# KLab/YAIK

Measured on AMD Instinct MI355X. Metric: Mpix/s tile encode (alpha reject + 7 gradient passes + 8x8 range quant), 8K RGBA, higher is better.
Workload: dtype u8/int32 (+f32 mode-selection sums)

## Files before the change

yaik_amd/csrc/yk_encode2.hip:

```cpp
#include "yk_common.h"
#include "yk_curves.h"
#include "yk_device.h"
#include <mutex>

__constant__ float c_curve2[6][16] = YK_CURVE_TABLE;

#define LS YK_LSTRIDE
#ifdef YK_TEST_HOOKS
#define YK2_ABLATE(bit) ((P.ablate & (bit)) != 0)
#else
#define YK2_ABLATE(bit) false
#endif

__device__ __forceinline__ int y2_byte(uint32_t w, int ch) { return (w >> (8 * ch)) & 255; }
__device__ __forceinline__ uint32_t y2_absdiff(uint32_t a, uint32_t b) { uint32_t r; asm("v_sad_u32 %0, %1, %2, 0" : "=v"(r) : "v"(a), "v"(b)); return r; }
__device__ __forceinline__ int y2_round6(int v) { return (v & ~3) | (v >> 6); }
__device__ __forceinline__ int y2_round6p(int v) { v = min(v + 1, 255); return (v & ~3) | (v >> 6); }

typedef short y2s2 __attribute__((ext_vector_type(2)));
typedef unsigned short y2u2 __attribute__((ext_vector_type(2)));
__device__ __forceinline__ y2u2 y2_u2(uint32_t w) { return __builtin_bit_cast(y2u2, w); }
__device__ __forceinline__ y2s2 y2_s2(y2u2 v) { return __builtin_bit_cast(y2s2, v); }
__device__ __forceinline__ y2u2 y2_splat(int v) { const unsigned short t = (unsigned short)v; return (y2u2){ t, t }; }
__device__ __forceinline__ y2s2 y2_splats(int v) { const short t = (short)v; return (y2s2){ t, t }; }
#define YK2_LATN 85
#ifdef YK2_STATS
__device__ unsigned long long g_y2_stats[128];
#define YK2_STAT(i, n) do { if (lane == 0) atomicAdd(&g_y2_stats[(i)], (unsigned long long)(n)); } while (0)
extern "C" int yk_debug_path_stats(unsigned long long* out, int clear) {
    hipError_t e = hipMemcpyFromSymbol(out, HIP_SYMBOL(g_y2_stats), sizeof(g_y2_stats));
    if (e == hipSuccess && clear) { static unsigned long long z[128]; e = hipMemcpyToSymbol(HIP_SYMBOL(g_y2_stats), z, sizeof(z)); }
    return (int)e;
}
#else
#define YK2_STAT(i, n) do { } while (0)
#endif

__device__ __forceinline__ constexpr int y2_cell_x(int m) { return (m & 1) | ((m >> 1) & 2); }
__device__ __forceinline__ constexpr int y2_cell_y(int m) { return ((m >> 1) & 1) | ((m >> 2) & 2); }
template <int NX, int NY> __device__ __forceinline__ constexpr unsigned long long y2_origin() {
    unsigned long long m = 0;
    for (int i = 0; i < 16; i++) if ((y2_cell_x(i) % NX) == 0 && (y2_cell_y(i) % NY) == 0) m |= 1ULL << i;
    return m * 0x0001000100010001ULL;
}
template <int NX, int NY> __device__ __forceinline__ unsigned long long y2_fold(unsigned long long m) {
    if (NX >= 2) m |= m >> 1;
    if (NY >= 2) m |= m >> 2;
    if (NX == 4) m |= m >> 4;
    if (NY == 4) m |= m >> 8;
    return m;
}
template <int NX, int NY> __device__ __forceinline__ unsigned long long y2_spread(unsigned long long m) {
    if (NX >= 2) m |= m << 1;
    if (NY >= 2) m |= m << 2;
    if (NX == 4) m |= m << 4;
    if (NY == 4) m |= m << 8;
    return m;
}

template <int SX, int SY, bool SMOOTH = false>
__device__ __forceinline__ void y2_grad_pass(const uint32_t* s_lat, const int lat, const int cx, const int cy,
                                             const uint32_t (&pwb)[16], unsigned long long& cov, const unsigned long long deadLanes, const bool stripInside,
                                             const int gxCell, const int gyCell, const int w, const int h, const int rf,
                                             uint32_t* s_bm, const int bxCell, const int byCell, const uint32_t* s_pix, uint8_t* s_list, uint32_t* s_tf, const int lane) {
    constexpr int TX = 1 << SX, TY = 1 << SY, NX = TX / 4, NY = TY / 4;
    constexpr unsigned long long ORG = y2_origin<NX, NY>();
    const int dcx = cx & (NX - 1), dcy = cy & (NY - 1);
    unsigned long long viable = ORG & ~cov & ~y2_fold<NX, NY>(deadLanes);
    if (!stripInside) {
        const int tgx = gxCell - dcx * 4, tgy = gyCell - dcy * 4;
        viable &= __ballot((tgx + TX <= w) && (tgy + TY <= h));
    }
    if (viable == 0ULL) return;
    constexpr int kPassId = (SX == 4 && SY == 4) ? 0 : (SX == 4 && SY == 3) ? 1 : (SX == 3 && SY == 4) ? 2 : (SX == 3 && SY == 3) ? 3 : (SX == 3 && SY == 2) ? 4 : (SX == 2 && SY == 3) ? 5 : 6;
    YK2_STAT(kPassId * 10 + 0, 1); YK2_STAT(kPassId * 10 + 8, __popcll(y2_spread<NX, NY>(viable)));
    const int loO = -256 * rf, hiO = 256 * rf + 255;
    const y2s2 loO2 = y2_splats(loO), hiO2 = y2_splats(hiO), loR2 = y2_splats(loO - 127), hiR2 = y2_splats(hiO - 127);


#ifndef YK2_NO_COMPACT
    const unsigned long long cells = y2_spread<NX, NY>(viable);
    const int nCells = __popcll(cells);
    if (nCells <= 16) {
        YK2_STAT(kPassId * 10 + 1, 1); YK2_STAT(kPassId * 10 + 7, nCells);
        const int rank = (int)__builtin_amdgcn_mbcnt_hi((uint32_t)(cells >> 32), __builtin_amdgcn_mbcnt_lo((uint32_t)cells, 0u));
        const bool mine = __builtin_amdgcn_inverse_ballot_w64(cells);
        if (mine) s_list[rank] = (uint8_t)lane;
        s_tf[lane] = 0u; s_tf[64 + lane] = 0u;
        __builtin_amdgcn_fence(__ATOMIC_RELEASE, "wavefront"); __builtin_amdgcn_wave_barrier(); __builtin_amdgcn_fence(__ATOMIC_ACQUIRE, "wavefront");
        const int j = lane & 15, r = lane >> 4;
        const bool act = j < nCells;
        const int c = (int)s_list[act ? j : 0];
        const int q2 = c >> 4, cy2 = y2_cell_y(c & 15), cx2 = y2_cell_x(c & 15);
        const int dcx2 = cx2 & (NX - 1), dcy2 = cy2 & (NY - 1);
        constexpr int kInTile = (NX > 1 ? 1 : 0) | (NY > 1 ? 2 : 0) | (NX > 2 ? 4 : 0) | (NY > 2 ? 8 : 0);
        const int orig = c & ~kInTile;
        const int lo2 = cy2 * 17 + q2 * 4 + cx2 - dcy2 * 17 - dcx2;
        const y2u2 wyr = y2_splat(16 - ((dcy2 * 4 + r) << (4 - SY)));
        const y2u2 lxc = y2_splat(16 - ((dcx2 * 4) << (4 - SX)));
        const uint4 pr = *reinterpret_cast<const uint4*>(&s_pix[(cy2 * 4 + r) * LS + q2 * 16 + cx2 * 4]);
        const uint32_t px[4] = { pr.x ^ 0x00808080u, pr.y ^ 0x00808080u, pr.z ^ 0x00808080u, pr.w ^ 0x00808080u };
        y2s2 mnc[5], mxc[5];
        auto rowC = [&](const unsigned mask) {
            y2u2 Sc[5], stc[5];
#pragma unroll
            for (int t = 0; t < 5; t++) {
                if (!((mask >> t) & 1u)) continue;
                const uint32_t* lt = s_lat + t * YK2_LATN + lo2;
                const y2u2 TL = y2_u2(lt[0]), TR = y2_u2(lt[NX]), BL = y2_u2(lt[NY * 17]), BR = y2_u2(lt[NY * 17 + NX]);
                const y2u2 e16 = (BL - BR) << 4, g = TR - BR, f = TL - BL - g;
                const y2u2 c2 = (g << 4) + f * lxc;
                Sc[t] = ((BR << 8) + e16 * lxc + c2 * wyr) ^ y2_splat(0x8000);
                stc[t] = (e16 + f * wyr) << (4 - SX);
            }
#pragma unroll
            for (int i = 0; i < 4; i++) {
                const uint32_t p = px[i];
                const y2s2 c01 = y2_s2(y2_u2(__builtin_amdgcn_perm(0u, p, 0x010C000Cu))), c22 = y2_s2(y2_u2(__builtin_amdgcn_perm(0u, p, 0x020C020Cu)));
                const y2s2 cc[4] = { __builtin_shufflevector(c01, c01, 0, 0), __builtin_shufflevector(c01, c01, 1, 1), c22, c01 };
#pragma unroll
                for (int t = 0; t < 5; t++) {
                    if (!((mask >> t) & 1u)) continue;
                    const y2s2 D = __builtin_elementwise_sub_sat(y2_s2(Sc[t]), cc[t == 4 ? 2 : t]);
                    if (i == 0) { mnc[t] = D; mxc[t] = D; }
                    else { mnc[t] = __builtin_elementwise_min(mnc[t], D); mxc[t] = __builtin_elementwise_max(mxc[t], D); }
                    if (i < 3) Sc[t] = Sc[t] - stc[t];
                }
            }
        };
        constexpr uint32_t kAllFail = 0xE000E000u;
        auto failBits = [&](const y2s2 mnA, const y2s2 mxA, const y2s2 mnP, const y2s2 mxP) -> uint32_t {
            const y2s2 zero = y2_splats(0);
            const y2s2 oA = __builtin_elementwise_sub_sat(zero, __builtin_elementwise_max(__builtin_elementwise_sub_sat(loO2, mnA), __builtin_elementwise_sub_sat(mxA, hiO2)));
            const y2s2 rA = __builtin_elementwise_sub_sat(zero, __builtin_elementwise_max(__builtin_elementwise_sub_sat(loR2, mnA), __builtin_elementwise_sub_sat(mxA, hiR2)));
            const y2s2 oP = __builtin_elementwise_sub_sat(zero, __builtin_elementwise_max(__builtin_elementwise_sub_sat(loO2, mnP), __builtin_elementwise_sub_sat(mxP, hiO2)));
            const y2s2 rP = __builtin_elementwise_sub_sat(zero, __builtin_elementwise_max(__builtin_elementwise_sub_sat(loR2, mnP), __builtin_elementwise_sub_sat(mxP, hiR2)));
            const uint32_t a = __builtin_bit_cast(uint32_t, oA), b = __builtin_bit_cast(uint32_t, rA), cO = __builtin_bit_cast(uint32_t, oP), cR = __builtin_bit_cast(uint32_t, rP);
            uint32_t m = (a & 0x80008000u) | ((b >> 1) & 0x40004000u);
            m |= (((cO << 16) | cO) >> 2) & 0x20000000u;
            m |= (((cR >> 16) | cR) >> 2) & 0x00002000u;
            return m;
        };
        rowC(0x09u);
        if (act) atomicOr(&s_tf[orig], failBits(mnc[0], mxc[0], mnc[3], mxc[3]));
        __builtin_amdgcn_fence(__ATOMIC_RELEASE, "wavefront"); __builtin_amdgcn_wave_barrier(); __builtin_amdgcn_fence(__ATOMIC_ACQUIRE, "wavefront");
        const unsigned long long alive = viable & __ballot(s_tf[lane] != kAllFail);
        if (alive == 0ULL) { YK2_STAT(100 + kPassId, 1); return; }
        rowC(0x16u);
        {
            const y2s2 mnA = __builtin_elementwise_min(__builtin_elementwise_min(mnc[0], mnc[1]), mnc[2]), mxA = __builtin_elementwise_max(__builtin_elementwise_max(mxc[0], mxc[1]), mxc[2]);
            const y2s2 mnP = __builtin_elementwise_min(mnc[3], mnc[4]), mxP = __builtin_elementwise_max(mxc[3], mxc[4]);
            if (act) atomicOr(&s_tf[64 + orig], failBits(mnA, mxA, mnP, mxP));
        }
        __builtin_amdgcn_fence(__ATOMIC_RELEASE, "wavefront"); __builtin_amdgcn_wave_barrier(); __builtin_amdgcn_fence(__ATOMIC_ACQUIRE, "wavefront");
        const unsigned long long acceptC = alive & __ballot(s_tf[64 + lane] != kAllFail);
        if (acceptC != 0ULL) {
            YK2_STAT(110 + kPassId, 1);
            cov |= y2_spread<NX, NY>(acceptC);
            if (__builtin_amdgcn_inverse_ballot_w64(acceptC)) {
                const int tbx = bxCell >> SX, tby = byCell >> SY;
                int bit;
                if (SX == 4 && SY == 4) bit = 0 + tby * 4 + tbx;
                else if (SX == 4 && SY == 3) bit = 32 + tby * 4 + tbx;
                else if (SX == 3 && SY == 4) bit = 64 + tby * 8 + tbx;
                else if (SX == 3 && SY == 3) bit = 96 + tby * 8 + tbx;
                else if (SX == 3 && SY == 2) bit = 160 + (tby >> 3) * 64 + (tby & 7) * 8 + tbx;
                else if (SX == 2 && SY == 3) bit = 288 + (tbx >> 3) * 64 + tby * 8 + (tbx & 7);
                else bit = 416 + ((tby >> 3) * 2 + (tbx >> 3)) * 64 + (tby & 7) * 8 + (tbx & 7);
                atomicOr(&s_bm[bit >> 5], 1u << (bit & 31));
            }
        }
        return;
    }
#endif

    const int lo = lat - dcy * 17 - dcx;
    const y2u2 wy2 = y2_splat(16 - ((dcy * 4) << (4 - SY)));
    const y2u2 lx2 = y2_splat(16 - ((dcx * 4) << (4 - SX)));
    y2u2 S[5], st[5], dS0[5], dS3[5], dst[5];
    auto setup = [&](const int t) {
        const uint32_t* lt = s_lat + t * YK2_LATN + lo;
        const y2u2 TL = y2_u2(lt[0]), TR = y2_u2(lt[NX]), BL = y2_u2(lt[NY * 17]), BR = y2_u2(lt[NY * 17 + NX]);
        const y2u2 e16 = (BL - BR) << 4, g = TR - BR, f = TL - BL - g;
        const y2u2 c2 = (g << 4) + f * lx2;
        S[t] = ((BR << 8) + e16 * lx2 + c2 * wy2) ^ y2_splat(0x8000);
        dS0[t] = c2 << (4 - SY);
        st[t] = (e16 + f * wy2) << (4 - SX);
        dst[t] = f << (8 - SX - SY);
        dS3[t] = dS0[t] - dst[t] * (unsigned short)3;
    };
    y2s2 mn[5], mx[5];
    auto pixelRow = [&](const int r, const unsigned mask, const bool first) {
#pragma unroll
        for (int ii = 0; ii < 4; ii++) {
            const int i = (r & 1) ? 3 - ii : ii;
            const uint32_t p = pwb[r * 4 + i];
            const y2s2 c01 = y2_s2(y2_u2(__builtin_amdgcn_perm(0u, p, 0x010C000Cu))), c22 = y2_s2(y2_u2(__builtin_amdgcn_perm(0u, p, 0x020C020Cu)));
            const y2s2 cc[4] = { __builtin_shufflevector(c01, c01, 0, 0), __builtin_shufflevector(c01, c01, 1, 1), c22, c01 };
#pragma unroll
            for (int t = 0; t < 5; t++) {
                if (!((mask >> t) & 1u)) continue;
                const y2s2 D = __builtin_elementwise_sub_sat(y2_s2(S[t]), cc[t == 4 ? 2 : t]);
                if (first && ii == 0) { mn[t] = D; mx[t] = D; }
                else { mn[t] = __builtin_elementwise_min(mn[t], D); mx[t] = __builtin_elementwise_max(mx[t], D); }
                if (ii < 3) S[t] = (r & 1) ? S[t] + st[t] : S[t] - st[t];
            }
        }
    };
    auto nextRow = [&](const int r, const unsigned mask) {
#pragma unroll
        for (int t = 0; t < 5; t++) if ((mask >> t) & 1u) { S[t] -= (r & 1) ? dS0[t] : dS3[t]; st[t] -= dst[t]; }
    };
    auto failA4 = [&](const y2s2 mnA, const y2s2 mxA) -> unsigned long long {
        const y2s2 oA = __builtin_elementwise_max(__builtin_elementwise_sub_sat(loO2, mnA), __builtin_elementwise_sub_sat(mxA, hiO2));
        const y2s2 rA = __builtin_elementwise_max(__builtin_elementwise_sub_sat(loR2, mnA), __builtin_elementwise_sub_sat(mxA, hiR2));
        unsigned long long f = y2_fold<NX, NY>(__ballot(oA.x > 0));
        f &= y2_fold<NX, NY>(__ballot(oA.y > 0));
        f &= y2_fold<NX, NY>(__ballot(rA.x > 0));
        f &= y2_fold<NX, NY>(__ballot(rA.y > 0));
        return f;
    };
    auto failP2 = [&](const y2s2 mnP, const y2s2 mxP) -> unsigned long long {
        const y2s2 oP = __builtin_elementwise_max(__builtin_elementwise_sub_sat(loO2, mnP), __builtin_elementwise_sub_sat(mxP, hiO2));
        const y2s2 rP = __builtin_elementwise_max(__builtin_elementwise_sub_sat(loR2, mnP), __builtin_elementwise_sub_sat(mxP, hiR2));
        return y2_fold<NX, NY>(__ballot((oP.x > 0) | (oP.y > 0))) & y2_fold<NX, NY>(__ballot((rP.x > 0) | (rP.y > 0)));
    };
    auto mnAll = [&]() { return __builtin_elementwise_min(__builtin_elementwise_min(mn[0], mn[1]), mn[2]); };
    auto mxAll = [&]() { return __builtin_elementwise_max(__builtin_elementwise_max(mx[0], mx[1]), mx[2]); };

    constexpr bool kScreen = (NX * NY >= 4);
    constexpr unsigned kA = 0x07u, kP = 0x18u;
    unsigned long long accept;
    if (SMOOTH) {
        setup(0); setup(1); setup(2);
        pixelRow(0, kA, true);
        nextRow(0, kA); pixelRow(1, kA, false);
        nextRow(1, kA); pixelRow(2, kA, false);
        nextRow(2, kA); pixelRow(3, kA, false);
        YK2_STAT(kPassId * 10 + 4, 1);
        accept = viable & ~failA4(mnAll(), mxAll());
#ifdef YK2_STATS
        {
            y2u2 S_[5], st_[5], a_[5], b_[5], c_[5]; y2s2 mn_[5], mx_[5];
            for (int t = 0; t < 5; t++) { S_[t] = S[t]; st_[t] = st[t]; a_[t] = dS0[t]; b_[t] = dS3[t]; c_[t] = dst[t]; mn_[t] = mn[t]; mx_[t] = mx[t]; }
            setup(3); setup(4);
            pixelRow(0, kP, true); nextRow(0, kP); pixelRow(1, kP, false); nextRow(1, kP); pixelRow(2, kP, false); nextRow(2, kP); pixelRow(3, kP, false);
            const unsigned long long accP = viable & ~failP2(__builtin_elementwise_min(mn[3], mn[4]), __builtin_elementwise_max(mx[3], mx[4]));
            YK2_STAT(97, __popcll(accept)); YK2_STAT(98, __popcll(accP)); YK2_STAT(99, __popcll(accept | accP)); YK2_STAT(96 + 0 * kPassId, 0);
            YK2_STAT(107, __popcll(viable));
            for (int t = 0; t < 5; t++) { S[t] = S_[t]; st[t] = st_[t]; dS0[t] = a_[t]; dS3[t] = b_[t]; dst[t] = c_[t]; mn[t] = mn_[t]; mx[t] = mx_[t]; }
        }
#endif
        const unsigned long long rest = viable & ~accept;
        if (rest != 0ULL) {
            YK2_STAT(kPassId * 10 + 5, 1); YK2_STAT(90 + kPassId, __popcll(y2_spread<NX, NY>(rest)));
            setup(3);
            pixelRow(0, 0x08u, true);
            const unsigned long long left = rest & ~failP2(mn[3], mx[3]);
            if (left != 0ULL) {
                setup(4);
                pixelRow(0, 0x10u, true);
                nextRow(0, kP); pixelRow(1, kP, false);
                nextRow(1, kP); pixelRow(2, kP, false);
                nextRow(2, kP); pixelRow(3, kP, false);
                accept |= left & ~failP2(__builtin_elementwise_min(mn[3], mn[4]), __builtin_elementwise_max(mx[3], mx[4]));
            }
        }
    } else {
    int pRows;
    if (kScreen) {
        setup(0); setup(3);
        pixelRow(0, 0x09u, true);
        viable &= ~(failA4(mn[0], mx[0]) & failP2(mn[3], mx[3]));
        if (viable == 0ULL) { YK2_STAT(kPassId * 10 + 2, 1); return; }
        setup(1); setup(2);
        pixelRow(0, 0x06u, true);
        viable &= ~(failA4(mnAll(), mxAll()) & failP2(mn[3], mx[3]));
        if (viable == 0ULL) { YK2_STAT(kPassId * 10 + 3, 1); return; }
        nextRow(0, kA);
        pixelRow(1, kA, false);
        pRows = 0;
    } else {
#pragma unroll
        for (int t = 0; t < 5; t++) setup(t);
        pixelRow(0, 0x1Fu, true);
        viable &= ~(failA4(mnAll(), mxAll()) & failP2(__builtin_elementwise_min(mn[3], mn[4]), __builtin_elementwise_max(mx[3], mx[4])));
        if (viable == 0ULL) { YK2_STAT(kPassId * 10 + 3, 1); return; }
        nextRow(0, 0x1Fu);
        pixelRow(1, 0x1Fu, false);
        if (NX * NY == 1) {
            viable &= ~(failA4(mnAll(), mxAll()) & failP2(__builtin_elementwise_min(mn[3], mn[4]), __builtin_elementwise_max(mx[3], mx[4])));
            if (viable == 0ULL) { YK2_STAT(kPassId * 10 + 9, 1); return; }
        }
        pRows = 2;
    }
    YK2_STAT(kPassId * 10 + 4, 1);
    nextRow(1, kA);
    pixelRow(2, kA, false);
    nextRow(2, kA);
    pixelRow(3, kA, false);
    accept = viable & ~failA4(mnAll(), mxAll());
    const unsigned long long rest = viable & ~accept;
    if (rest != 0ULL) {
        YK2_STAT(kPassId * 10 + 5, 1); YK2_STAT(90 + kPassId, __popcll(y2_spread<NX, NY>(rest)));
        if (kScreen) {
            setup(4);
            pixelRow(0, 0x10u, true);
            nextRow(0, kP);
            pixelRow(1, kP, false);
        }
        nextRow(1, kP);
        pixelRow(2, kP, false);
        nextRow(2, kP);
        pixelRow(3, kP, false);
        accept |= rest & ~failP2(__builtin_elementwise_min(mn[3], mn[4]), __builtin_elementwise_max(mx[3], mx[4]));
    }
    (void)pRows;
    }
    if (accept == 0ULL) return;
    YK2_STAT(kPassId * 10 + 6, 1);
    cov |= y2_spread<NX, NY>(accept);
    if (__builtin_amdgcn_inverse_ballot_w64(accept)) {
        const int tbx = bxCell >> SX, tby = byCell >> SY;
        int bit;
        if (SX == 4 && SY == 4) bit = 0 + tby * 4 + tbx;
        else if (SX == 4 && SY == 3) bit = 32 + tby * 4 + tbx;
        else if (SX == 3 && SY == 4) bit = 64 + tby * 8 + tbx;
        else if (SX == 3 && SY == 3) bit = 96 + tby * 8 + tbx;
        else if (SX == 3 && SY == 2) bit = 160 + (tby >> 3) * 64 + (tby & 7) * 8 + tbx;
        else if (SX == 2 && SY == 3) bit = 288 + (tbx >> 3) * 64 + tby * 8 + (tbx & 7);
        else bit = 416 + ((tby >> 3) * 2 + (tbx >> 3)) * 64 + (tby & 7) * 8 + (tbx & 7);
        atomicOr(&s_bm[bit >> 5], 1u << (bit & 31));
    }
}

#define YK2_QROWS 258
#define YK2_QR0 32
#define YK2_QNR 224
#define YK2_QBYTES ((size_t)YK2_QNR * YK2_QROWS * 16)
#define YK2_RCPBYTES ((size_t)256 * sizeof(float))
#define YK2_DEFN1 224
#define YK2_DEFBYTES ((size_t)225 * YK2_DEFN1 * 4)
#define YK2_TABBYTES (YK2_QBYTES + YK2_RCPBYTES + YK2_DEFBYTES)
typedef _Float16 y2h2 __attribute__((ext_vector_type(2)));
__device__ __forceinline__ uint32_t y2_f16_bits(int n) { const _Float16 h = (_Float16)(float)n; return (uint32_t)__builtin_bit_cast(unsigned short, h); }
__global__ void yk_qtab_kernel(uint4* tab) {
    __shared__ int K[6][16];
    const int R = YK2_QR0 + (int)blockIdx.x, t = threadIdx.x;
    if (t < 96) { const int m = t >> 4, i = t & 15; K[m][i] = __float2int_rz(__fmul_rn(c_curve2[m][i], (float)R)); }
    __syncthreads();
    if (t < YK2_QROWS) {
        const int o = t - 2;
        uint32_t md[6], idx = 0;
        for (int m = 0; m < 6; m++) {
            const int cnt = m < 3 ? 16 : 8;
            int best = 1 << 30, bi = 0;
            for (int n = 0; n < cnt; n++) { const int d = abs(K[m][n] - o); if (d < best) { best = d; bi = n; } }
            best = min(best, 255);
            md[m] = y2_f16_bits(best);
            idx |= (uint32_t)bi << (4 * m);
        }
        tab[(size_t)blockIdx.x * YK2_QROWS + t] = make_uint4(md[0] | (md[1] << 16), md[2] | (md[3] << 16), md[4] | (md[5] << 16), idx);
    }
}
struct Y2TileDef { int base, BN, dist, R; };
__device__ __forceinline__ Y2TileDef y2_tile_def(const int min_, const int d8) {
    Y2TileDef d;
    d.base = (min_ * 63 + 112) / 224;
    d.BN = (d.base * 224) / 63;
    const int scale = 223 - d.BN;
    const int dnum = (d8 - 32) * 127 + (scale - 1);
    d.dist = (scale < 0) ? -dnum : dnum / scale;
    d.R = (d.dist * scale) / 127 + 32;
// ... 193 lines not shown
            Rb = *reinterpret_cast<const int4*>(b0 + off);
            Gb = *reinterpret_cast<const int4*>(b1 + off);
            Bb = *reinterpret_cast<const int4*>(b2 + off);
        }
        uint32_t hcol;
        const int hr = min(max(lane - 32, 0), 16);
        {
            const int rel = min(gyS + hr, P.hAvail - 1) - gyB;
            const uint32_t off = (uint32_t)(rel * P.strideElems + min(BX * 64 + 64, w - 1)) * 4u;
            hcol = y2_pack3(*reinterpret_cast<const int32_t*>(b0 + off), *reinterpret_cast<const int32_t*>(b1 + off), *reinterpret_cast<const int32_t*>(b2 + off));
        }
        const float4 rc4 = *reinterpret_cast<const float4*>(P.qtab + YK2_QBYTES + (size_t)lane * 16);

        __builtin_amdgcn_s_setprio(0);
        uint4 o[4], ob;
#pragma unroll
        for (int k = 0; k < 4; k++) {
            o[k] = make_uint4(y2_pack3(R[k].x, G[k].x, B[k].x), y2_pack3(R[k].y, G[k].y, B[k].y), y2_pack3(R[k].z, G[k].z, B[k].z), y2_pack3(R[k].w, G[k].w, B[k].w));
            *reinterpret_cast<uint4*>(&s_pix[(r0 + 4 * k) * LS + g4]) = o[k];
        }
        ob = make_uint4(y2_pack3(Rb.x, Gb.x, Bb.x), y2_pack3(Rb.y, Gb.y, Bb.y), y2_pack3(Rb.z, Gb.z, Bb.z), y2_pack3(Rb.w, Gb.w, Bb.w));
        if (lane < 16) *reinterpret_cast<uint4*>(&s_pix[16 * LS + g4]) = ob;
        if (BX * 64 + 64 > w) {
            if (!inX) {
#pragma unroll
                for (int k = 0; k < 4; k++) *reinterpret_cast<uint4*>(&s_pix[(r0 + 4 * k) * LS + g4]) = make_uint4(o[k].w, o[k].w, o[k].w, o[k].w);
                if (lane < 16) *reinterpret_cast<uint4*>(&s_pix[16 * LS + g4]) = make_uint4(ob.w, ob.w, ob.w, ob.w);
            }
        }
        if (lane >= 32 && lane <= 48) s_pix[hr * LS + 64] = hcol;
        *reinterpret_cast<float4*>(&s_rcp[lane * 4]) = rc4;

    }
    __syncthreads();
    YK2_PROBE(1);

    const int q = lane >> 4, cx = y2_cell_x(lane & 15), cy = y2_cell_y(lane & 15);
    const int bxCell = q * 16 + cx * 4, byCell = wave * 16 + cy * 4;
    const int gxCell = BX * 64 + bxCell, gyCell = BY * 64 + byCell;
    const int lcell = (cy * 4) * LS + bxCell;
    const int lat = cy * 17 + q * 4 + cx;
    const bool mtIn = (BX * 64 + q * 16 < w) && (BY * 64 + wave * 16 < h);

    uint32_t pw[16];
#pragma unroll
    for (int r = 0; r < 4; r++) {
        const uint4 t = *reinterpret_cast<const uint4*>(&s_pix[lcell + r * LS]);
        pw[r * 4 + 0] = t.x; pw[r * 4 + 1] = t.y; pw[r * 4 + 2] = t.z; pw[r * 4 + 3] = t.w;
    }

    unsigned long long cov = 0ULL;
    {
        bool dead = !mtIn;
        {
            const int lim = 4 * P.rejectFactor + 1;
            const y2u2 rb0 = y2_u2(pw[0] & 0x00FF00FFu), rb1 = y2_u2(pw[1] & 0x00FF00FFu), rb2 = y2_u2(pw[2] & 0x00FF00FFu), rb3 = y2_u2(pw[3] & 0x00FF00FFu);
            const y2u2 ga = y2_u2(__builtin_amdgcn_perm(pw[1], pw[0], 0x0C050C01u)), gb = y2_u2(__builtin_amdgcn_perm(pw[2], pw[1], 0x0C050C01u)),
                       gc = y2_u2(__builtin_amdgcn_perm(pw[3], pw[2], 0x0C050C01u));
            const y2u2 l2 = y2_splat(lim);
            const y2u2 u1 = rb0 + rb2 - rb1 - rb1 + l2, u2 = rb1 + rb3 - rb2 - rb2 + l2, ug = ga + gc - gb - gb + l2;
            const y2u2 um = __builtin_elementwise_max(__builtin_elementwise_max(u1, u2), ug);
            dead |= __builtin_bit_cast(uint32_t, __builtin_elementwise_sub_sat(um, y2_splat(2 * lim))) != 0u;
        }
        const unsigned long long deadLanes = __ballot(dead);
        YK2_STAT(75, 1); YK2_STAT(76, ~deadLanes == 0ULL ? 1 : 0); YK2_STAT(77, __popcll(deadLanes));
        const bool stripInside = (BX * 64 + 64 <= w) && (BY * 64 + wave * 16 + 16 <= h);
        if (~deadLanes != 0ULL && !YK2_ABLATE(2)) {
            auto latticePoint = [&](const int idx) {
                const int lr = (idx * 241) >> 12, lc = idx - lr * 17;
                const uint32_t raw = s_pix[(lr * 4) * LS + lc * 4];
                const uint32_t r6 = (raw & 0x00FCFCFCu) | ((raw >> 6) & 0x00030303u);
                const uint32_t z = (raw & 0x007F7F7Fu) + 0x00010101u;
                const uint32_t inc = (z ^ (raw & 0x00808080u)) | (((z & raw & 0x00808080u) >> 7) * 255u);
                const uint32_t p6 = (inc & 0x00FCFCFCu) | ((inc >> 6) & 0x00030303u);
                s_lat[0 * YK2_LATN + idx] = __builtin_amdgcn_perm(r6, raw, 0x0C040C00u);
                s_lat[1 * YK2_LATN + idx] = __builtin_amdgcn_perm(r6, raw, 0x0C050C01u);
                s_lat[2 * YK2_LATN + idx] = __builtin_amdgcn_perm(r6, raw, 0x0C060C02u);
                s_lat[3 * YK2_LATN + idx] = __builtin_amdgcn_perm(p6, p6, 0x0C010C00u);
                s_lat[4 * YK2_LATN + idx] = __builtin_amdgcn_perm(p6, p6, 0x0C020C02u);
            };
            latticePoint(lane);
            if (lane < YK2_LATN - 64) latticePoint(lane + 64);
            __syncthreads();
#pragma unroll
            for (int k = 0; k < 16; k++) pw[k] ^= 0x00808080u;
            if (deadLanes == 0ULL) y2_grad_pass<4, 4, true>(s_lat, lat, cx, cy, pw, cov, deadLanes, stripInside, gxCell, gyCell, w, h, P.rejectFactor, s_bm, bxCell, byCell, s_pix, s_list, s_range, lane);
            else y2_grad_pass<4, 4>(s_lat, lat, cx, cy, pw, cov, deadLanes, stripInside, gxCell, gyCell, w, h, P.rejectFactor, s_bm, bxCell, byCell, s_pix, s_list, s_range, lane);
            if (~(cov | deadLanes) != 0ULL) {
                y2_grad_pass<4, 3>(s_lat, lat, cx, cy, pw, cov, deadLanes, stripInside, gxCell, gyCell, w, h, P.rejectFactor, s_bm, bxCell, byCell, s_pix, s_list, s_range, lane);
                y2_grad_pass<3, 4>(s_lat, lat, cx, cy, pw, cov, deadLanes, stripInside, gxCell, gyCell, w, h, P.rejectFactor, s_bm, bxCell, byCell, s_pix, s_list, s_range, lane);
                y2_grad_pass<3, 3>(s_lat, lat, cx, cy, pw, cov, deadLanes, stripInside, gxCell, gyCell, w, h, P.rejectFactor, s_bm, bxCell, byCell, s_pix, s_list, s_range, lane);
                y2_grad_pass<3, 2>(s_lat, lat, cx, cy, pw, cov, deadLanes, stripInside, gxCell, gyCell, w, h, P.rejectFactor, s_bm, bxCell, byCell, s_pix, s_list, s_range, lane);
                y2_grad_pass<2, 3>(s_lat, lat, cx, cy, pw, cov, deadLanes, stripInside, gxCell, gyCell, w, h, P.rejectFactor, s_bm, bxCell, byCell, s_pix, s_list, s_range, lane);
                y2_grad_pass<2, 2>(s_lat, lat, cx, cy, pw, cov, deadLanes, stripInside, gxCell, gyCell, w, h, P.rejectFactor, s_bm, bxCell, byCell, s_pix, s_list, s_range, lane);
            }
#pragma unroll
            for (int k = 0; k < 16; k++) pw[k] ^= 0x00808080u;
        }
    }
    const int mtIdx = ((BY * 64 + wave * 16) >> 4) * P.mtW + ((BX * 64 + q * 16) >> 4);
    __syncthreads();
    YK2_PROBE(2);
    uint8_t* const small = P.small;
    const uint32_t bmv = s_bm[lane < 24 ? lane : 0];
    auto bmWord = [&](const int k) -> uint32_t { return (uint32_t)__builtin_amdgcn_readlane((int)bmv, k); };
    const uint32_t i64 = (uint32_t)(BY * P.xBB64 + BX);
    const uint32_t frU = (uint32_t)fr;
    uint32_t off32 = ~0u, val32 = 0u;
    {
        const uint32_t w1 = (uint32_t)wave & 1u, w2 = (uint32_t)wave >> 1;
        uint32_t off8 = 0u, val8 = 0u;
        off8 = y2_writelane(P.oBm0b + frU * (uint32_t)P.fs.bm0b + i64 * 4u + (uint32_t)wave, 0, off8);
        val8 = y2_writelane((bmWord(0) >> (4 * wave)) & 0xFu, 0, val8);
        off8 = y2_writelane(P.oBm[1] + frU * (uint32_t)P.fs.bitmap[1] + i64 * 4u + (uint32_t)wave, 1, off8);
        val8 = y2_writelane(bmWord(1) >> (8 * wave), 1, val8);
        off8 = y2_writelane(P.oBm[2] + frU * (uint32_t)P.fs.bitmap[2] + i64 * 4u + (uint32_t)wave, 2, off8);
        val8 = y2_writelane(bmWord(2) >> (8 * wave), 2, val8);
        if (lane < 3) Y2_STORE_IF(8, *(small + off8), (uint8_t)val8);
        const unsigned long long t = ((cov >> 2) ^ cov) & 0x0C0C0C0C0C0C0C0CULL;
        const unsigned long long covRM = cov ^ t ^ (t << 2);
        uint32_t off16 = ((lane & 15) == 0 && mtIn) ? P.oCov + (frU * (uint32_t)P.fs.coverage + (uint32_t)mtIdx) * 2u : ~0u;
        uint32_t val16 = (uint32_t)((covRM >> (q * 16)) & 0xFFFFULL);
        off16 = y2_writelane(P.oBm[3] + frU * (uint32_t)P.fs.bitmap[3] + (i64 * 4u + (uint32_t)wave) * 2u, 1, off16);
        val16 = y2_writelane(bmWord(3 + (int)w2) >> (16 * w1), 1, val16);
#pragma unroll
        for (int sx = 0; sx < 2; sx++) {
            const bool in = BX * 2 + sx < P.xBB32;
            off16 = y2_writelane(in ? P.oBm[5] + frU * (uint32_t)P.fs.bitmap[5] + ((uint32_t)((BY * P.xBB32 + BX * 2 + sx) * 4 + wave)) * 2u : ~0u, 2 + sx, off16);
            val16 = y2_writelane(bmWord(9 + sx * 2 + (int)w2) >> (16 * w1), 2 + sx, val16);
        }
        if (off16 != ~0u) Y2_STORE_IF(8, *reinterpret_cast<uint16_t*>(small + off16), (uint16_t)val16);
        if (P.pixCache != nullptr) {
            const bool cellIn = (gxCell < w) && (gyCell < h);
            if (cellIn && !((cov >> lane) & 1ULL)) {
                const uint32_t strip = (uint32_t)((BY * 4 + wave) * P.xBB64 + BX);
                uint4* dstp = P.pixCache + (size_t)strip * 256 + lane;
#pragma unroll
                for (int r = 0; r < 4; r++) dstp[r * 64] = make_uint4(pw[r * 4 + 0], pw[r * 4 + 1], pw[r * 4 + 2], pw[r * 4 + 3]);
            }
        }
        {
            const bool in = BY * 2 + (int)w2 < P.yBB32;
            off32 = y2_writelane(in ? P.oBm[4] + frU * (uint32_t)P.fs.bitmap[4] + ((uint32_t)(((BY * 2 + (int)w2) * P.xBB64 + BX) * 2) + w1) * 4u : ~0u, 1, off32);
            val32 = y2_writelane(bmWord(5 + (int)w2 * 2 + (int)w1), 1, val32);
#pragma unroll
            for (int sx = 0; sx < 2; sx++) {
                const bool in6 = in && (BX * 2 + sx < P.xBB32);
                off32 = y2_writelane(in6 ? P.oBm[6] + frU * (uint32_t)P.fs.bitmap[6] + ((uint32_t)(((BY * 2 + (int)w2) * P.xBB32 + BX * 2 + sx) * 2) + w1) * 4u : ~0u, 2 + sx, off32);
                val32 = y2_writelane(bmWord(13 + ((int)w2 * 2 + sx) * 2 + (int)w1), 2 + sx, val32);
            }
        }
    }
    YK2_PROBE(3);
    int cxB = 0, cyB = 0, cw = w, chh = P.fullH, discard = 1;
    if (boundsP) {
        const int b0 = boundsP[0], b1 = boundsP[1], b2 = boundsP[2], b3 = boundsP[3];
        discard = (b0 == 0 && b1 == 0 && b2 == w && b3 == P.fullH) ? 1 : 0;
        cxB = (b0 >> 3) << 3; cyB = (b1 >> 3) << 3;
        cw = (((b2 + 7) >> 3) << 3) - cxB; chh = (((b3 + 7) >> 3) << 3) - cyB;
    }
    const int cxl = cx & 1, cyl = cy & 1;
    const int tgx = gxCell - cxl * 4, tgyl = gyCell - cyl * 4, tgy = tgyl + P.y0;
    const bool tileIn = (tgx + 8 <= w) && (tgyl + 8 <= h);
    const bool part = tileIn && tgx >= cxB && tgx < cxB + cw && tgy >= cyB && tgy < cyB + chh && (tgx + 8 <= cw) && (tgy + 8 <= chh);
    const bool keepMT = (keepP == nullptr) || discard || (mtIn && keepP[mtIdx] != 0);
    const bool tileLive = part && keepMT;
    const int l00 = lane & ~3;
    const uint32_t quadN = (uint32_t)((~cov) >> l00) & 15u;
    const int v00 = (int)(quadN & 1u), v01 = (int)((quadN >> 2) & 1u);
    const bool valid = tileLive && ((quadN >> (lane & 3)) & 1u);
    const int nTop = __popc(quadN & 3u), nBot = __popc(quadN >> 2);
    const int tileIdx = (tgyl >> 3) * P.tilesW + (tgx >> 3);
    const size_t T8 = (size_t)P.tilesW * P.tilesH;
    const int tw = lane >> 2;
    const bool writer = ((lane & 3) == 0) && tileIn;
    const unsigned long long validMask = __ballot(valid);
#ifdef YK2_NO_WIDE_STORE
    const bool fullTiles = false;
#else
    const bool fullTiles = !WANT_DST && __ballot(tileLive && quadN != 15u && quadN != 0u) == 0ULL;
// ... 418 lines not shown
```

Baseline: 227,800.

## Pre-unpack pixel channels once and pack blue-channel pass two pixels per lane

Pixels are unpacked into signed 16-bit RG and paired-blue vectors once per tile and passed to every gradient pass, so each pass no longer repeats the perm/xor unpack. The fifth term (blue, which was duplicated) is now evaluated for two pixels per packed op, using precomputed per-half start and row-step values, which halves its per-pixel instruction count. The early two-row reject check is extended to passes with NX*NY equal to 2. The cost is extra registers for the 24 pre-unpacked vectors plus a reload of pw from LDS afterwards, which may raise VGPR pressure and lower occupancy.

```diff
diff --git a/yaik_amd/csrc/yk_encode2.hip b/yaik_amd/csrc/yk_encode2.hip
--- a/yaik_amd/csrc/yk_encode2.hip
+++ b/yaik_amd/csrc/yk_encode2.hip
@@ -23,6 +23,8 @@
 __device__ __forceinline__ y2s2 y2_s2(y2u2 v) { return __builtin_bit_cast(y2s2, v); }
 __device__ __forceinline__ y2u2 y2_splat(int v) { const unsigned short t = (unsigned short)v; return (y2u2){ t, t }; }
 __device__ __forceinline__ y2s2 y2_splats(int v) { const short t = (short)v; return (y2s2){ t, t }; }
+__device__ __forceinline__ y2s2 y2_rg(uint32_t p) { return y2_s2(y2_u2(__builtin_amdgcn_perm(0u, p, 0x010C000Cu) ^ 0x80008000u)); }
+__device__ __forceinline__ y2s2 y2_bb(uint32_t pEven, uint32_t pOdd) { return y2_s2(y2_u2(__builtin_amdgcn_perm(pOdd, pEven, 0x060C020Cu) ^ 0x80008000u)); }
 #define YK2_LATN 85
 #ifdef YK2_STATS
 __device__ unsigned long long g_y2_stats[128];
@@ -60,7 +62,7 @@
 
 template <int SX, int SY, bool SMOOTH = false>
 __device__ __forceinline__ void y2_grad_pass(const uint32_t* s_lat, const int lat, const int cx, const int cy,
-                                             const uint32_t (&pwb)[16], unsigned long long& cov, const unsigned long long deadLanes, const bool stripInside,
+                                             const y2s2 (&rg)[16], const y2s2 (&bb)[8], unsigned long long& cov, const unsigned long long deadLanes, const bool stripInside,
                                              const int gxCell, const int gyCell, const int w, const int h, const int rf,
                                              uint32_t* s_bm, const int bxCell, const int byCell, const uint32_t* s_pix, uint8_t* s_list, uint32_t* s_tf, const int lane) {
     constexpr int TX = 1 << SX, TY = 1 << SY, NX = TX / 4, NY = TY / 4;
@@ -99,7 +101,7 @@
         const y2u2 wyr = y2_splat(16 - ((dcy2 * 4 + r) << (4 - SY)));
         const y2u2 lxc = y2_splat(16 - ((dcx2 * 4) << (4 - SX)));
         const uint4 pr = *reinterpret_cast<const uint4*>(&s_pix[(cy2 * 4 + r) * LS + q2 * 16 + cx2 * 4]);
-        const uint32_t px[4] = { pr.x ^ 0x00808080u, pr.y ^ 0x00808080u, pr.z ^ 0x00808080u, pr.w ^ 0x00808080u };
+        const y2s2 rgc[4] = { y2_rg(pr.x), y2_rg(pr.y), y2_rg(pr.z), y2_rg(pr.w) }, bbc[2] = { y2_bb(pr.x, pr.y), y2_bb(pr.z, pr.w) };
         y2s2 mnc[5], mxc[5];
         auto rowC = [&](const unsigned mask) {
             y2u2 Sc[5], stc[5];
@@ -115,17 +117,22 @@
             }
 #pragma unroll
             for (int i = 0; i < 4; i++) {
-                const uint32_t p = px[i];
-                const y2s2 c01 = y2_s2(y2_u2(__builtin_amdgcn_perm(0u, p, 0x010C000Cu))), c22 = y2_s2(y2_u2(__builtin_amdgcn_perm(0u, p, 0x020C020Cu)));
-                const y2s2 cc[4] = { __builtin_shufflevector(c01, c01, 0, 0), __builtin_shufflevector(c01, c01, 1, 1), c22, c01 };
-#pragma unroll
-                for (int t = 0; t < 5; t++) {
+                const y2s2 c01 = rgc[i], cb = bbc[i >> 1];
+                const y2s2 cc[4] = { __builtin_shufflevector(c01, c01, 0, 0), __builtin_shufflevector(c01, c01, 1, 1),
+                                     (i & 1) ? __builtin_shufflevector(cb, cb, 1, 1) : __builtin_shufflevector(cb, cb, 0, 0), c01 };
+#pragma unroll
+                for (int t = 0; t < 4; t++) {
                     if (!((mask >> t) & 1u)) continue;
-                    const y2s2 D = __builtin_elementwise_sub_sat(y2_s2(Sc[t]), cc[t == 4 ? 2 : t]);
+                    const y2s2 D = __builtin_elementwise_sub_sat(y2_s2(Sc[t]), cc[t]);
                     if (i == 0) { mnc[t] = D; mxc[t] = D; }
                     else { mnc[t] = __builtin_elementwise_min(mnc[t], D); mxc[t] = __builtin_elementwise_max(mxc[t], D); }
                     if (i < 3) Sc[t] = Sc[t] - stc[t];
                 }
+            }
+            if (mask & 0x10u) {
+                const y2s2 Da = __builtin_elementwise_sub_sat(y2_s2(Sc[4] - stc[4] * (y2u2){ 0, 1 }), bbc[0]);
+                const y2s2 Db = __builtin_elementwise_sub_sat(y2_s2(Sc[4] - stc[4] * (y2u2){ 2, 3 }), bbc[1]);
+                mnc[4] = __builtin_elementwise_min(Da, Db); mxc[4] = __builtin_elementwise_max(Da, Db);
             }
         };
         constexpr uint32_t kAllFail = 0xE000E000u;
@@ -177,39 +184,55 @@
     const int lo = lat - dcy * 17 - dcx;
     const y2u2 wy2 = y2_splat(16 - ((dcy * 4) << (4 - SY)));
     const y2u2 lx2 = y2_splat(16 - ((dcx * 4) << (4 - SX)));
-    y2u2 S[5], st[5], dS0[5], dS3[5], dst[5];
+    y2u2 S[4], st[4], dS0[4], dS3[4], dst[4], Sa, Sb, rsA, rsB;
     auto setup = [&](const int t) {
         const uint32_t* lt = s_lat + t * YK2_LATN + lo;
         const y2u2 TL = y2_u2(lt[0]), TR = y2_u2(lt[NX]), BL = y2_u2(lt[NY * 17]), BR = y2_u2(lt[NY * 17 + NX]);
         const y2u2 e16 = (BL - BR) << 4, g = TR - BR, f = TL - BL - g;
         const y2u2 c2 = (g << 4) + f * lx2;
-        S[t] = ((BR << 8) + e16 * lx2 + c2 * wy2) ^ y2_splat(0x8000);
-        dS0[t] = c2 << (4 - SY);
-        st[t] = (e16 + f * wy2) << (4 - SX);
-        dst[t] = f << (8 - SX - SY);
-        dS3[t] = dS0[t] - dst[t] * (unsigned short)3;
+        const y2u2 s0 = ((BR << 8) + e16 * lx2 + c2 * wy2) ^ y2_splat(0x8000);
+        const y2u2 d0 = c2 << (4 - SY);
+        const y2u2 sx = (e16 + f * wy2) << (4 - SX);
+        const y2u2 dx = f << (8 - SX - SY);
+        if (t < 4) {
+            S[t] = s0; dS0[t] = d0; st[t] = sx; dst[t] = dx;
+            dS3[t] = d0 - dx * (unsigned short)3;
+        } else {
+            const y2u2 k01 = { 0, 1 }, k23 = { 2, 3 };
+            Sa = s0 - sx * k01; Sb = s0 - sx * k23;
+            rsA = d0 - dx * k01; rsB = d0 - dx * k23;
+        }
     };
     y2s2 mn[5], mx[5];
     auto pixelRow = [&](const int r, const unsigned mask, const bool first) {
-#pragma unroll
-        for (int ii = 0; ii < 4; ii++) {
-            const int i = (r & 1) ? 3 - ii : ii;
-            const uint32_t p = pwb[r * 4 + i];
-            const y2s2 c01 = y2_s2(y2_u2(__builtin_amdgcn_perm(0u, p, 0x010C000Cu))), c22 = y2_s2(y2_u2(__builtin_amdgcn_perm(0u, p, 0x020C020Cu)));
-            const y2s2 cc[4] = { __builtin_shufflevector(c01, c01, 0, 0), __builtin_shufflevector(c01, c01, 1, 1), c22, c01 };
-#pragma unroll
-            for (int t = 0; t < 5; t++) {
-                if (!((mask >> t) & 1u)) continue;
-                const y2s2 D = __builtin_elementwise_sub_sat(y2_s2(S[t]), cc[t == 4 ? 2 : t]);
-                if (first && ii == 0) { mn[t] = D; mx[t] = D; }
-                else { mn[t] = __builtin_elementwise_min(mn[t], D); mx[t] = __builtin_elementwise_max(mx[t], D); }
-                if (ii < 3) S[t] = (r & 1) ? S[t] + st[t] : S[t] - st[t];
-            }
+        if (mask & 0x0Fu) {
+#pragma unroll
+            for (int ii = 0; ii < 4; ii++) {
+                const int i = (r & 1) ? 3 - ii : ii;
+                const y2s2 c01 = rg[r * 4 + i], cb = bb[r * 2 + (i >> 1)];
+                const y2s2 cc[4] = { __builtin_shufflevector(c01, c01, 0, 0), __builtin_shufflevector(c01, c01, 1, 1),
+                                     (i & 1) ? __builtin_shufflevector(cb, cb, 1, 1) : __builtin_shufflevector(cb, cb, 0, 0), c01 };
+#pragma unroll
+                for (int t = 0; t < 4; t++) {
+                    if (!((mask >> t) & 1u)) continue;
+                    const y2s2 D = __builtin_elementwise_sub_sat(y2_s2(S[t]), cc[t]);
+                    if (first && ii == 0) { mn[t] = D; mx[t] = D; }
+                    else { mn[t] = __builtin_elementwise_min(mn[t], D); mx[t] = __builtin_elementwise_max(mx[t], D); }
+                    if (ii < 3) S[t] = (r & 1) ? S[t] + st[t] : S[t] - st[t];
+                }
+            }
+        }
+        if (mask & 0x10u) {
+            const y2s2 Da = __builtin_elementwise_sub_sat(y2_s2(Sa), bb[r * 2]), Db = __builtin_elementwise_sub_sat(y2_s2(Sb), bb[r * 2 + 1]);
+            const y2s2 lo4 = __builtin_elementwise_min(Da, Db), hi4 = __builtin_elementwise_max(Da, Db);
+            if (first) { mn[4] = lo4; mx[4] = hi4; }
+            else { mn[4] = __builtin_elementwise_min(mn[4], lo4); mx[4] = __builtin_elementwise_max(mx[4], hi4); }
         }
     };
     auto nextRow = [&](const int r, const unsigned mask) {
 #pragma unroll
-        for (int t = 0; t < 5; t++) if ((mask >> t) & 1u) { S[t] -= (r & 1) ? dS0[t] : dS3[t]; st[t] -= dst[t]; }
+        for (int t = 0; t < 4; t++) if ((mask >> t) & 1u) { S[t] -= (r & 1) ? dS0[t] : dS3[t]; st[t] -= dst[t]; }
+        if (mask & 0x10u) { Sa -= rsA; Sb -= rsB; }
     };
     auto failA4 = [&](const y2s2 mnA, const y2s2 mxA) -> unsigned long long {
         const y2s2 oA = __builtin_elementwise_max(__builtin_elementwise_sub_sat(loO2, mnA), __builtin_elementwise_sub_sat(mxA, hiO2));
@@ -241,14 +264,16 @@
         accept = viable & ~failA4(mnAll(), mxAll());
 #ifdef YK2_STATS
         {
-            y2u2 S_[5], st_[5], a_[5], b_[5], c_[5]; y2s2 mn_[5], mx_[5];
-            for (int t = 0; t < 5; t++) { S_[t] = S[t]; st_[t] = st[t]; a_[t] = dS0[t]; b_[t] = dS3[t]; c_[t] = dst[t]; mn_[t] = mn[t]; mx_[t] = mx[t]; }
+            y2u2 S_[4], st_[4], a_[4], b_[4], c_[4]; y2s2 mn_[5], mx_[5];
+            for (int t = 0; t < 4; t++) { S_[t] = S[t]; st_[t] = st[t]; a_[t] = dS0[t]; b_[t] = dS3[t]; c_[t] = dst[t]; }
+            for (int t = 0; t < 5; t++) { mn_[t] = mn[t]; mx_[t] = mx[t]; }
             setup(3); setup(4);
             pixelRow(0, kP, true); nextRow(0, kP); pixelRow(1, kP, false); nextRow(1, kP); pixelRow(2, kP, false); nextRow(2, kP); pixelRow(3, kP, false);
             const unsigned long long accP = viable & ~failP2(__builtin_elementwise_min(mn[3], mn[4]), __builtin_elementwise_max(mx[3], mx[4]));
             YK2_STAT(97, __popcll(accept)); YK2_STAT(98, __popcll(accP)); YK2_STAT(99, __popcll(accept | accP)); YK2_STAT(96 + 0 * kPassId, 0);
             YK2_STAT(107, __popcll(viable));
-            for (int t = 0; t < 5; t++) { S[t] = S_[t]; st[t] = st_[t]; dS0[t] = a_[t]; dS3[t] = b_[t]; dst[t] = c_[t]; mn[t] = mn_[t]; mx[t] = mx_[t]; }
+            for (int t = 0; t < 4; t++) { S[t] = S_[t]; st[t] = st_[t]; dS0[t] = a_[t]; dS3[t] = b_[t]; dst[t] = c_[t]; }
+            for (int t = 0; t < 5; t++) { mn[t] = mn_[t]; mx[t] = mx_[t]; }
         }
 #endif
         const unsigned long long rest = viable & ~accept;
@@ -288,7 +313,7 @@
         if (viable == 0ULL) { YK2_STAT(kPassId * 10 + 3, 1); return; }
         nextRow(0, 0x1Fu);
         pixelRow(1, 0x1Fu, false);
-        if (NX * NY == 1) {
+        if (NX * NY <= 2) {
             viable &= ~(failA4(mnAll(), mxAll()) & failP2(__builtin_elementwise_min(mn[3], mn[4]), __builtin_elementwise_max(mx[3], mx[4])));
             if (viable == 0ULL) { YK2_STAT(kPassId * 10 + 9, 1); return; }
         }
@@ -648,20 +673,26 @@
             latticePoint(lane);
             if (lane < YK2_LATN - 64) latticePoint(lane + 64);
             __syncthreads();
-#pragma unroll
-            for (int k = 0; k < 16; k++) pw[k] ^= 0x00808080u;
-            if (deadLanes == 0ULL) y2_grad_pass<4, 4, true>(s_lat, lat, cx, cy, pw, cov, deadLanes, stripInside, gxCell, gyCell, w, h, P.rejectFactor, s_bm, bxCell, byCell, s_pix, s_list, s_range, lane);
-            else y2_grad_pass<4, 4>(s_lat, lat, cx, cy, pw, cov, deadLanes, stripInside, gxCell, gyCell, w, h, P.rejectFactor, s_bm, bxCell, byCell, s_pix, s_list, s_range, lane);
+            y2s2 rg[16], bb[8];
+#pragma unroll
+            for (int k = 0; k < 16; k++) rg[k] = y2_rg(pw[k]);
+#pragma unroll
+            for (int k = 0; k < 8; k++) bb[k] = y2_bb(pw[2 * k], pw[2 * k + 1]);
+            if (deadLanes == 0ULL) y2_grad_pass<4, 4, true>(s_lat, lat, cx, cy, rg, bb, cov, deadLanes, stripInside, gxCell, gyCell, w, h, P.rejectFactor, s_bm, bxCell, byCell, s_pix, s_list, s_range, lane);
+            else y2_grad_pass<4, 4>(s_lat, lat, cx, cy, rg, bb, cov, deadLanes, stripInside, gxCell, gyCell, w, h, P.rejectFactor, s_bm, bxCell, byCell, s_pix, s_list, s_range, lane);
             if (~(cov | deadLanes) != 0ULL) {
-                y2_grad_pass<4, 3>(s_lat, lat, cx, cy, pw, cov, deadLanes, stripInside, gxCell, gyCell, w, h, P.rejectFactor, s_bm, bxCell, byCell, s_pix, s_list, s_range, lane);
-                y2_grad_pass<3, 4>(s_lat, lat, cx, cy, pw, cov, deadLanes, stripInside, gxCell, gyCell, w, h, P.rejectFactor, s_bm, bxCell, byCell, s_pix, s_list, s_range, lane);
-                y2_grad_pass<3, 3>(s_lat, lat, cx, cy, pw, cov, deadLanes, stripInside, gxCell, gyCell, w, h, P.rejectFactor, s_bm, bxCell, byCell, s_pix, s_list, s_range, lane);
-                y2_grad_pass<3, 2>(s_lat, lat, cx, cy, pw, cov, deadLanes, stripInside, gxCell, gyCell, w, h, P.rejectFactor, s_bm, bxCell, byCell, s_pix, s_list, s_range, lane);
-                y2_grad_pass<2, 3>(s_lat, lat, cx, cy, pw, cov, deadLanes, stripInside, gxCell, gyCell, w, h, P.rejectFactor, s_bm, bxCell, byCell, s_pix, s_list, s_range, lane);
-                y2_grad_pass<2, 2>(s_lat, lat, cx, cy, pw, cov, deadLanes, stripInside, gxCell, gyCell, w, h, P.rejectFactor, s_bm, bxCell, byCell, s_pix, s_list, s_range, lane);
-            }
-#pragma unroll
-            for (int k = 0; k < 16; k++) pw[k] ^= 0x00808080u;
+                y2_grad_pass<4, 3>(s_lat, lat, cx, cy, rg, bb, cov, deadLanes, stripInside, gxCell, gyCell, w, h, P.rejectFactor, s_bm, bxCell, byCell, s_pix, s_list, s_range, lane);
+                y2_grad_pass<3, 4>(s_lat, lat, cx, cy, rg, bb, cov, deadLanes, stripInside, gxCell, gyCell, w, h, P.rejectFactor, s_bm, bxCell, byCell, s_pix, s_list, s_range, lane);
+                y2_grad_pass<3, 3>(s_lat, lat, cx, cy, rg, bb, cov, deadLanes, stripInside, gxCell, gyCell, w, h, P.rejectFactor, s_bm, bxCell, byCell, s_pix, s_list, s_range, lane);
+                y2_grad_pass<3, 2>(s_lat, lat, cx, cy, rg, bb, cov, deadLanes, stripInside, gxCell, gyCell, w, h, P.rejectFactor, s_bm, bxCell, byCell, s_pix, s_list, s_range, lane);
+                y2_grad_pass<2, 3>(s_lat, lat, cx, cy, rg, bb, cov, deadLanes, stripInside, gxCell, gyCell, w, h, P.rejectFactor, s_bm, bxCell, byCell, s_pix, s_list, s_range, lane);
+                y2_grad_pass<2, 2>(s_lat, lat, cx, cy, rg, bb, cov, deadLanes, stripInside, gxCell, gyCell, w, h, P.rejectFactor, s_bm, bxCell, byCell, s_pix, s_list, s_range, lane);
+            }
+#pragma unroll
+            for (int r = 0; r < 4; r++) {
+                const uint4 t = *reinterpret_cast<const uint4*>(&s_pix[lcell + r * LS]);
+                pw[r * 4 + 0] = t.x; pw[r * 4 + 1] = t.y; pw[r * 4 + 2] = t.z; pw[r * 4 + 3] = t.w;
+            }
         }
     }
     const int mtIdx = ((BY * 64 + wave * 16) >> 4) * P.mtW + ((BX * 64 + q * 16) >> 4);
```

Measured after the change: 234,600, median of 6. 3.0% higher.
